# sayands/sgaligner

Hardware: AMD Instinct MI355X
Metric: subscan-pairs/sec (fwd+bwd) + node-match Hits@1 vs reference (higher is better)
Workload: dtype f32 (fp32 operands and fp32 accumulation throughout; the anchors x negatives loss sweeps multiply them as three exact bf16 planes, six bf16 MFMAs per product...

## Files before the change

sgaligner_amd/csrc/sweep3.hip:

```cpp
#include <type_traits>

#include "loss_math.h"

namespace {

typedef __bf16 bf16x8 __attribute__((ext_vector_type(8)));
typedef __bf16 bf16x2 __attribute__((ext_vector_type(2)));
typedef float f32x2 __attribute__((ext_vector_type(2)));
typedef unsigned int u32x4 __attribute__((ext_vector_type(4)));
typedef unsigned int u32x2 __attribute__((ext_vector_type(2)));
typedef short s16x4 __attribute__((ext_vector_type(4)));

constexpr int S3_DP = 104;
constexpr int S3_PLANE = 3 * 2 * 1024;
constexpr int S3_TAIL = 3 * S3_PLANE;
constexpr int S3_BLOCK = S3_TAIL + 2048;
constexpr int S3_NCH = S3_BLOCK / 1024;
constexpr int S3_ROWSLOTS = 3 * 12 + 4;

__device__ __forceinline__ void split3_pair(float v0, float v1, unsigned& h, unsigned& m, unsigned& l) {
    const bf16x2 H = __builtin_convertvector(f32x2{v0, v1}, bf16x2);
    const unsigned hu = __builtin_bit_cast(unsigned, H);
#ifdef S3_SPLIT_DOT2
    unsigned c0 = 0x0000BF80u, c1 = 0xBF800000u;
// ... 82 lines not shown
    if (b < L.nbA) { old0 = 0; len = A; }
    else if (b < 2 * L.nbA) { b -= L.nbA; old0 = A; len = A; }
    else if (b < 2 * L.nbA + L.nb1) { b -= 2 * L.nbA; old0 = 2 * A; len = J1; }
    else { b -= 2 * L.nbA + L.nb1; old0 = 2 * A + J1; len = J2; }
    const int nvalid = min(32, len - 32 * b);
    const float* src = Z + (size_t)(old0 + 32 * b) * S3_DP;
    if (threadIdx.x < S3_DP) zbar[threadIdx.x] = stat[threadIdx.x];
    __syncthreads();
    for (int e = threadIdx.x; e < 32 * S3_DP; e += 256) {
        const int r = e / S3_DP, c = e - r * S3_DP;
        tile[e] = (r < nvalid && c < S3_DREAL) ? src[e] - zbar[c] : 0.f;
        if (Zc && old0 < 2 * A && r < nvalid) Zc[(size_t)(old0 + 32 * b) * S3_DP + e] = c == S3_DREAL + 1 ? 1.f : tile[e];
    }
    __syncthreads();
    if (threadIdx.x < 32) {
        const int r = threadIdx.x;
        if (r < nvalid) {
            double a = 0.0;
            for (int c = 0; c < S3_DREAL; ++c) a += (double)zbar[c] * (double)tile[r * S3_DP + c];
            tile[r * S3_DP + S3_DREAL] = (float)(a + (double)stat[S3_DP]);
            tile[r * S3_DP + S3_DREAL + 1] = 1.f;
        }
    }
    __syncthreads();
    unsigned* out = reinterpret_cast<unsigned*>(Zb + (size_t)blockIdx.x * S3_BLOCK);
    for (int e = threadIdx.x; e < 3 * 2 * 64 * 4; e += 256) {
        const int p = e & 3, st = (e >> 2) & 63, jh = (e >> 8) & 1, q = e >> 9;
        const int g = st >> 4, i = (st & 15) ^ (12 * (g & 1));
        const int row = 8 * (i >> 2) + 4 * jh + (i & 3), col = 32 * q + 8 * g + 2 * p;
        unsigned h, m, l;
        split3_pair(tile[row * S3_DP + col], tile[row * S3_DP + col + 1], h, m, l);
        out[e] = h; out[S3_PLANE / 4 + e] = m; out[2 * S3_PLANE / 4 + e] = l;
    }
    for (int e = threadIdx.x; e < 2 * 64 * 4; e += 256) {
        const int p = e & 3, st = (e >> 2) & 63, jh = (e >> 8) & 1;
        const int g = st >> 4, i = (st & 15) ^ (12 * (g & 1));
        const int row = 8 * (i >> 2) + 4 * jh + (i & 3), col = 96 + 2 * p;
        unsigned h, m, l;
        split3_pair(tile[row * S3_DP + col], tile[row * S3_DP + col + 1], h, m, l);
        out[S3_TAIL / 4 + e] = g < 2 ? h : (g == 2 ? m : l);
    }
}


__global__ __launch_bounds__(256) void centre_tables_kernel(const float* __restrict__ Z, int R, const float* __restrict__ stat, float* __restrict__ Zc) {
    const int lane = threadIdx.x & 63, wpb = blockDim.x >> 6;
    for (int r = blockIdx.x * wpb + (threadIdx.x >> 6); r < R; r += gridDim.x * wpb) {
        const float* z = Z + (size_t)r * S3_DP;
        float* o = Zc + (size_t)r * S3_DP;
        double acc = 0.0;
        float v[2];
#pragma unroll
        for (int t = 0; t < 2; ++t) {
            const int d = lane + 64 * t;
            const float zb = d < S3_DREAL ? stat[d] : 0.f;
            v[t] = d < S3_DREAL ? z[d] - zb : 0.f;
            acc += (double)zb * (double)v[t];
        }
        acc = wave_sum_d(acc);
        o[lane] = v[0];
        const int d1 = lane + 64;
        if (d1 < S3_DP) o[d1] = d1 < S3_DREAL ? v[1] : (d1 == S3_DREAL ? (float)(acc + (double)stat[S3_DP]) : (d1 == S3_DREAL + 1 ? 1.f : 0.f));
    }
}

#ifdef S3_DBG_TIMING
__device__ unsigned long long g_s3_dbg[16];
#define S3_T(i) { const unsigned long long t_ = __builtin_readcyclecounter(); tacc[i] += t_ - tprev; tprev = t_; }
#else
#define S3_T(i)
#endif
struct TSeg { int blk0, jt_lo, jt_hi, old0, lo, hi, fam; };
struct TGroup { int own0, nown, own_old0, own_blk0, blk0, nsplit, nseg; TSeg seg[2]; };
struct TArgs {
    int M; const unsigned char* Zb[4]; int perm[4]; int ngroups; TGroup grp[4];
    float k0, k1, it0, it1, ka;
    const float* beta;
    double* sums;
    const double* gs;
    float* dZ[4];
    double* gamma;
};

template <int M, bool GRAD, int WV, int MG = M, bool GAM = true, bool LITE = false, bool FOLD = false>
__global__ __launch_bounds__(WV * 64, WV == 8 ? 2 : 1) void sweep3_kernel(TArgs a) {
    static_assert(!LITE || !GRAD, "LITE: the forward sums only");
    static_assert(!FOLD || (GRAD && WV == 4), "FOLD: the one-wave-per-SIMD gradient sweep only");
    constexpr int NCT = 7;
    constexpr int WAVES = WV, THREADS = WAVES * 64;
    constexpr int OWN = WV * 16;
    constexpr int NCH = LITE ? S3_NCH - S3_PLANE / 1024 : S3_NCH;
    constexpr int KMAX = (NCH + WAVES - 1) / WAVES;
    constexpr int BUF = M * S3_BLOCK;
    constexpr bool PIPE = WV == 4;
#ifndef S3_OWN_IN_S
#define S3_OWN_IN_S 1
#endif
    constexpr bool OWN_IN_S = GRAD && PIPE && S3_OWN_IN_S;
#ifndef S3_SPREAD
#define S3_SPREAD 1
#endif
    constexpr bool SPREAD = OWN_IN_S && S3_SPREAD && !FOLD;
    extern __shared__ __attribute__((aligned(16))) unsigned char lds3[];

    const int tid = threadIdx.x, lane = tid & 63, wave = tid >> 6, g4 = lane >> 4, l15 = lane & 15;
    int g = 0;
#pragma unroll
    for (int i = 1; i < 4; ++i) if (i < a.ngroups && (int)blockIdx.x >= a.grp[i].blk0) g = i;
    const TGroup& grp = a.grp[g];
    const int wg_in_grp = (int)blockIdx.x - grp.blk0;
    const int nsplit = grp.nsplit, n_ob = (grp.nown + OWN - 1) / OWN, n_units = n_ob * nsplit;
    const int unit = (wg_in_grp & 7) * ((n_units + 7) >> 3) + (wg_in_grp >> 3);
    if ((wg_in_grp >> 3) >= ((n_units + 7) >> 3) || unit >= n_units) return;
    const int split = unit / n_ob;
    const int own0 = grp.own0 + (unit - split * n_ob) * OWN;
    const int own_end = grp.own0 + grp.nown;
    const int wrow0 = own0 + wave * 16;
#ifdef S3_DBG_TIMING
    unsigned long long tacc[8] = {0, 0, 0, 0, 0, 0, 0, 0}, tprev = __builtin_readcyclecounter();
#endif

    u32x4 opl[M][3][3], otl[M][2];
    float beta[M];
    const bool iv = wrow0 + l15 < own_end;
    {
        const int my_i = wrow0 + l15;
        const int rel = (iv ? my_i : own0) - grp.own_old0;
        const int o = rel & 31, oi = 4 * (o >> 3) + (o & 3), ojh = (o >> 2) & 1;
        const size_t off = (size_t)(grp.own_blk0 + (rel >> 5)) * S3_BLOCK;
#pragma unroll
        for (int m = 0; m < M; ++m) {
            const unsigned char* base = a.Zb[m] + off;
#pragma unroll
            for (int p = 0; p < 3; ++p)
#pragma unroll
                for (int q = 0; q < 3; ++q) {
                    const int so = ((q * 2 + ojh) * 64 + s3_slot(g4, oi)) * 16;
                    opl[m][p][q] = iv ? *reinterpret_cast<const u32x4*>(base + p * S3_PLANE + so) : u32x4{0, 0, 0, 0};
                }
            u32x4 th = iv ? *reinterpret_cast<const u32x4*>(base + S3_TAIL + (ojh * 64 + s3_slot(0, oi)) * 16) : u32x4{0, 0, 0, 0};
            u32x4 tm = iv ? *reinterpret_cast<const u32x4*>(base + S3_TAIL + (ojh * 64 + s3_slot(2, oi)) * 16) : u32x4{0, 0, 0, 0};
            u32x4 tl = iv ? *reinterpret_cast<const u32x4*>(base + S3_TAIL + (ojh * 64 + s3_slot(3, oi)) * 16) : u32x4{0, 0, 0, 0};
            const float ksc = a.k1;
            auto rescale = [&](u32x4& ph, u32x4& pm, u32x4& pl) {
#pragma unroll
                for (int d = 0; d < 4; ++d) {
                    const float x0 = (__builtin_bit_cast(float, ph[d] << 16) + __builtin_bit_cast(float, pm[d] << 16)) + __builtin_bit_cast(float, pl[d] << 16);
                    const float x1 = (__builtin_bit_cast(float, ph[d] & 0xffff0000u) + __builtin_bit_cast(float, pm[d] & 0xffff0000u)) + __builtin_bit_cast(float, pl[d] & 0xffff0000u);
                    unsigned nh, nm, nl;
                    split3_pair(x0 * ksc, x1 * ksc, nh, nm, nl);
                    ph[d] = nh; pm[d] = nm; pl[d] = nl;
                }
            };
#pragma unroll
            for (int q = 0; q < 3; ++q) rescale(opl[m][0][q], opl[m][1][q], opl[m][2][q]);
            rescale(th, tm, tl);
            otl[m][0] = g4 == 1 ? tm : th;
            otl[m][1] = g4 == 0 ? tl : (g4 == 2 ? tm : u32x4{0, 0, 0, 0});
#pragma unroll
            for (int t = 0; t < 2; ++t)
                otl[m][t][2] = (otl[m][t][2] >> 16) | (otl[m][t][2] << 16);
        }
    }
#pragma unroll
    for (int m = 0; m < M; ++m) beta[m] = a.beta[a.perm[m]];

    constexpr int NSM = GRAD ? (FOLD ? 1 : MG) : 1;
    f32x4 gacc[GRAD ? MG : 1][NCT], gsm[NSM][NCT];
#pragma unroll
    for (int m = 0; m < (GRAD ? MG : 1); ++m)
#pragma unroll
        for (int ct = 0; ct < NCT; ++ct) gacc[m][ct] = f32x4{0.f, 0.f, 0.f, 0.f};
#pragma unroll
    for (int m = 0; m < NSM; ++m)
#pragma unroll
        for (int ct = 0; ct < NCT; ++ct) gsm[m][ct] = f32x4{0.f, 0.f, 0.f, 0.f};
    float gam[M];
#pragma unroll
    for (int m = 0; m < M; ++m) gam[m] = 0.f;

    const int wave_u = __builtin_amdgcn_readfirstlane(wave);
    unsigned l16 = threadIdx.x;
    asm volatile("" : "+v"(l16));
    l16 = (l16 & 63u) * 16u;
    unsigned long long tb[M];
    auto set_tile = [&](int blk) {
#pragma unroll
        for (int m = 0; m < M; ++m) tb[m] = sreg64(reinterpret_cast<unsigned long long>(a.Zb[m]) + (unsigned long long)blk * S3_BLOCK);
    };
    auto issue_slots = [&](unsigned char* buf, int f_lo, int f_hi) {
#ifdef S3_DBG_NODMA
        return;
#endif
#pragma unroll
        for (int f = f_lo; f < f_hi; ++f) {
            if (f >= M * KMAX) break;
            const int m = f / KMAX, k = f % KMAX;
            const int rot = (wave_u + m) & (WAVES - 1);
            int c = rot + k * WAVES;
            if ((k + 1) * WAVES > NCH) c = c >= NCH ? c - WAVES : c;
            if (LITE) c = c >= 2 * (S3_PLANE / 1024) ? c + S3_PLANE / 1024 : c;
            __builtin_amdgcn_global_load_lds((const __attribute__((address_space(1))) void*)(reinterpret_cast<const unsigned char*>(tb[m] + (unsigned)(c * 1024)) + l16),
                                             (__attribute__((address_space(3))) void*)(buf + m * S3_BLOCK + c * 1024), 16, 0, 0);
        }
    };
    auto issue = [&](int blk, unsigned char* buf) { set_tile(blk); issue_slots(buf, 0, M * KMAX); };

    const int aoff = s3_slot(g4, l15) * 16;
    const int tr_io = 4 * g4 + (l15 >> 2), tr_cs = l15 & 3;
    const int tr_main = s3_slot(tr_cs >> 1, tr_io) * 16 + (tr_cs & 1) * 8;
    const int tr_tail = S3_TAIL + tr_io * 16 + (tr_cs & 1) * 8;
    const int tr_tail_l = S3_TAIL + (48 + (tr_io ^ 12)) * 16 + (tr_cs & 1) * 8;

#pragma unroll 1
    for (int sg = 0; sg < 2; ++sg) {
        if (sg >= grp.nseg) break;
        const TSeg seg = grp.seg[sg];
        float c0[M + 1], c1[M + 1];
#pragma unroll
        for (int m = 0; m <= M; ++m) {
            const int mo = m < M ? a.perm[m] : M;
            c0[m] = GRAD ? (float)(a.gs[mo * 8 + seg.fam * 2 + 0] * (double)a.it0) : 0.f;
            c1[m] = GRAD ? (float)(a.gs[mo * 8 + seg.fam * 2 + 1] * (double)a.it1) : 0.f;
        }
        const float ka = a.ka;
        double dsum[M + 1][2];
#pragma unroll
        for (int m = 0; m <= M; ++m) { dsum[m][0] = 0.0; dsum[m][1] = 0.0; }
        float pl0[LITE ? M + 1 : 1], pl1[LITE ? M + 1 : 1];
#pragma unroll
        for (int m = 0; m < (LITE ? M + 1 : 1); ++m) { pl0[m] = 0.f; pl1[m] = 0.f; }

        __syncthreads();
        if (seg.jt_lo + split < seg.jt_hi) issue(seg.blk0 + seg.jt_lo + split, lds3);
        int it = 0;
#pragma unroll 1
        for (int jt = seg.jt_lo + split; jt < seg.jt_hi; jt += nsplit, ++it) {
            unsigned char* buf = lds3 + (it & 1) * BUF;
            const int j0 = seg.old0 + 32 * jt;
            S3_T(5)
            __syncthreads();
            S3_T(0)
            const int next_blk = seg.blk0 + (jt + nsplit < seg.jt_hi ? jt + nsplit : jt);
            unsigned char* next_buf = lds3 + ((it + 1) & 1) * BUF;
            set_tile(next_blk);
            S3_T(1)
            if (GRAD) {
                const int vlo = max(seg.lo - j0, 0), vhi = min(seg.hi - j0, 32);
                if (vlo > 0 || vhi < 32) {
                    for (int x = tid; x < M * 32 * S3_ROWSLOTS; x += THREADS) {
                        const int pc = x % S3_ROWSLOTS, w = (x / S3_ROWSLOTS) % 32, m = x / (S3_ROWSLOTS * 32);
                        if (w >= vlo && w < vhi) continue;
                        const int wjh = (w >> 2) & 1, wi = 4 * (w >> 3) + (w & 3);
                        unsigned char* base = buf + m * S3_BLOCK;
                        if (pc < 36) {
                            const int pl = pc / 12, q = (pc % 12) >> 2, gq = pc & 3;
                            *reinterpret_cast<u32x4*>(base + pl * S3_PLANE + ((q * 2 + wjh) * 64 + s3_slot(gq, wi)) * 16) = u32x4{0, 0, 0, 0};
                        } else {
                            const int gq = pc - 36;
                            *reinterpret_cast<u32x4*>(base + S3_TAIL + (wjh * 64 + s3_slot(gq, wi)) * 16) = u32x4{0, 0, 0, 0};
                        }
                    }
                    __syncthreads();
                }
            }

            f32x4 sacc[M][2];
            float own[M][2][4];
            float cj[2][4];
            constexpr int NSET = PIPE ? 2 : 1;
            u32x4 at[NSET], ap[NSET][3][3];
            auto ld_one = [&](int ss, int idx) {
                const int e = ss % NSET;
                const unsigned char* ar = buf + (SPREAD ? ss % M : ss >> 1) * S3_BLOCK + (SPREAD ? ss / M : ss & 1) * 1024 + aoff;
                if (idx < 1) at[e] = *reinterpret_cast<const u32x4*>(ar + S3_TAIL);
                else ap[e][2 - (idx - 1) / 3][(idx - 1) % 3] = *reinterpret_cast<const u32x4*>(ar + (2 - (idx - 1) / 3) * S3_PLANE + ((idx - 1) % 3) * 2048);
            };
            auto ld_set = [&](int ss) {
#pragma unroll
                for (int idx = 0; idx < 10; ++idx) if (!(LITE && idx >= 1 && idx <= 3)) ld_one(ss, idx);
            };
            if (PIPE) {
                ld_set(0);
                __builtin_amdgcn_s_waitcnt(0xc07f);
                __builtin_amdgcn_sched_barrier(0);
            }
            if constexpr (SPREAD) {
                constexpr int NDS = 2 * M - 2, PER = (M * KMAX + NDS - 1) / NDS;
                constexpr int PA[6] = {2, 1, 1, 0, 0, 0}, PB[6] = {0, 1, 0, 2, 1, 0};
                f32x4 accp[2][2];
                float ot0 = 0.f, ot1 = 0.f, sjt = 0.f, ce0 = 0.f, ce1 = 0.f;
                auto own_step = [&](int mm, int hh, int r, int k) {
                    const float sv = sacc[mm][hh][r];
                    if (k == 0) ot0 = fexp2(sv * ka);
                    else if (k == 1) ot1 = fexp2(sv);
                    else own[mm][hh][r] = fmaf(c0[mm], ot0, c1[mm] * ot1);
                };
                auto cj_step = [&](int hh, int r, int k) {
                    if (k == 0) {
                        sjt = 0.f;
#pragma unroll
                        for (int mm = 0; mm < M; ++mm) sjt = fmaf(beta[mm], sacc[mm][hh][r], sjt);
                    } else if (k == 1) ce0 = fexp2(sjt * ka);
                    else if (k == 2) ce1 = fexp2(sjt);
                    else cj[hh][r] = c0[M] * ce0 + c1[M] * ce1;
                };
#pragma unroll
                for (int ss = 0; ss < 2 * M; ++ss) {
                    const int m = ss % M, jh = ss / M, e = ss % NSET, pa = ss & 1;
                    const int pm = ss > 0 ? (ss - 1) % M : 0, pjh = ss > 0 ? (ss - 1) / M : 0;
                    accp[pa][0] = f32x4{0.f, 0.f, 0.f, 0.f}; accp[pa][1] = f32x4{0.f, 0.f, 0.f, 0.f};
#pragma unroll
                    for (int x = 0; x < 20; ++x) {
                        if (x == 0) accp[pa][0] = mfma_b(at[e], otl[m][1], accp[pa][0]);
                        else if (x == 1) accp[pa][1] = mfma_b(at[e], otl[m][0], accp[pa][1]);
                        else accp[pa][x & 1] = mfma_b(ap[e][PA[(x - 2) / 3]][(x - 2) % 3], opl[m][PB[(x - 2) / 3]][(x - 2) % 3], accp[pa][x & 1]);
                        __builtin_amdgcn_sched_barrier(0);
                        if (ss + 1 < 2 * M && x < 10) ld_one(ss + 1, x);
                        if (ss < NDS && (x % 3) == 1 && (x / 3) < PER) issue_slots(next_buf, ss * PER + (x / 3), ss * PER + (x / 3) + 1);
                        if (ss > 0) {
                            if (x == 0) { sacc[pm][pjh][0] = accp[pa ^ 1][0][0] + accp[pa ^ 1][1][0]; sacc[pm][pjh][1] = accp[pa ^ 1][0][1] + accp[pa ^ 1][1][1]; }
                            if (x == 2) { sacc[pm][pjh][2] = accp[pa ^ 1][0][2] + accp[pa ^ 1][1][2]; sacc[pm][pjh][3] = accp[pa ^ 1][0][3] + accp[pa ^ 1][1][3]; }
                            if (pm < MG) {
                                constexpr int G0[4] = {3, 8, 12, 16}, G1[4] = {5, 9, 14, 17}, G2[4] = {6, 11, 15, 18};
#pragma unroll
                                for (int r = 0; r < 4; ++r) {
                                    if (x == G0[r]) own_step(pm, pjh, r, 0);
                                    if (x == G1[r]) own_step(pm, pjh, r, 1);
                                    if (x == G2[r]) own_step(pm, pjh, r, 2);
                                }
                            }
                        }
                        if (ss >= NDS) {
                            const int q = (x == 19 ? 5 : (x % 3) == 1 && x <= 13 ? x / 3 : -1);
                            if (q >= 0) {
                                const int qq = (ss - NDS) * 6 + q, r = qq / 3, k = qq % 3;
                                if (k == 0) { if (r > 0) cj_step(0, r - 1, 3); cj_step(0, r, 0); }
                                else cj_step(0, r, k);
                            }
                        }
                        __builtin_amdgcn_sched_barrier(0);
                    }
                }
#pragma unroll
                for (int r = 0; r < 4; ++r) sacc[M - 1][1][r] = accp[(2 * M - 1) & 1][0][r] + accp[(2 * M - 1) & 1][1][r];
                cj_step(0, 3, 3);
            } else {
#pragma unroll
            for (int ss = 0; ss < 2 * M; ++ss) {
                const int m = ss >> 1, jh = ss & 1, e = ss % NSET;
                if (!PIPE) ld_set(ss);
                constexpr int NDS = GRAD ? (2 * M - 2) : 2 * M, PER = (M * KMAX + NDS - 1) / NDS;
                f32x4 acc2[2] = {f32x4{0.f, 0.f, 0.f, 0.f}, f32x4{0.f, 0.f, 0.f, 0.f}};
                float ownt[2] = {0.f, 0.f};
                constexpr int PA[6] = {2, 1, 1, 0, 0, 0}, PB[6] = {0, 1, 0, 2, 1, 0};
#pragma unroll
                for (int x = 0; x < 20; ++x) {
                    const bool skip = LITE && x >= 2 && (PA[(x - 2) / 3] == 2 || PB[(x - 2) / 3] == 2 || (PA[(x - 2) / 3] == 1 && PB[(x - 2) / 3] == 1));
                    if (skip) {}
                    else if (x == 0) acc2[0] = mfma_b(at[e], otl[m][1], acc2[0]);
                    else if (x == 1) acc2[1] = mfma_b(at[e], otl[m][0], acc2[1]);
                    else acc2[x & 1] = mfma_b(ap[e][PA[(x - 2) / 3]][(x - 2) % 3], opl[m][PB[(x - 2) / 3]][(x - 2) % 3], acc2[x & 1]);
                    if (PIPE) {
                        __builtin_amdgcn_sched_barrier(0);
                        if (ss + 1 < 2 * M && x < 10 && !(LITE && x >= 1 && x <= 3)) ld_one(ss + 1, x);
                        if (ss < NDS && (x % 3) == 1 && (x / 3) < PER) issue_slots(next_buf, ss * PER + (x / 3), ss * PER + (x / 3) + 1);
                        if (OWN_IN_S && m > 0 && m - 1 < MG && x >= 11 && x < 19) {
                            const int r = (x - 11) >> 1;
                            const float sv = sacc[m - 1][jh][r];
                            if (((x - 11) & 1) == 0) {
                                ownt[0] = fexp2(sv * ka);
                                ownt[1] = fexp2(sv);
                            } else {
                                own[m - 1][jh][r] = fmaf(c0[m - 1], ownt[0], c1[m - 1] * ownt[1]);
                            }
                        }
                        __builtin_amdgcn_sched_barrier(0);
                    } else if (x == 1 && ss < NDS) {
                        issue_slots(next_buf, ss * PER, (ss + 1) * PER);
                    }
                }
#pragma unroll
                for (int r = 0; r < 4; ++r) sacc[m][jh][r] = acc2[0][r] + acc2[1][r];
            }
            }

            S3_T(2)
            if (!GRAD) {
                float p0[M + 1], p1[M + 1];
#pragma unroll
                for (int m = 0; m <= M; ++m) { p0[m] = LITE ? pl0[LITE ? m : 0] : 0.f; p1[m] = LITE ? pl1[LITE ? m : 0] : 0.f; }
                auto sums_tile = [&](auto masked_c) {
                    constexpr bool MASKED = decltype(masked_c)::value;
#pragma unroll
                    for (int jh = 0; jh < 2; ++jh)
#pragma unroll
                        for (int r = 0; r < 4; ++r) {
                            const int row = j0 + 8 * g4 + 4 * jh + r;
                            const float okf = (!MASKED || (iv && row >= seg.lo && row < seg.hi)) ? 1.f : 0.f;
                            float sj = 0.f;
#pragma unroll
                            for (int m = 0; m < M; ++m) {
                                const float sv = sacc[m][jh][r];
                                sj = fmaf(beta[m], sv, sj);
                                p0[m] = MASKED ? fmaf(okf, fexp2(sv * ka), p0[m]) : p0[m] + fexp2(sv * ka);
                                p1[m] = MASKED ? fmaf(okf, fexp2(sv), p1[m]) : p1[m] + fexp2(sv);
                            }
                            p0[M] = MASKED ? fmaf(okf, fexp2(sj * ka), p0[M]) : p0[M] + fexp2(sj * ka);
                            p1[M] = MASKED ? fmaf(okf, fexp2(sj), p1[M]) : p1[M] + fexp2(sj);
                        }
                };
                if (j0 >= seg.lo && j0 + 32 <= seg.hi && own0 + OWN <= own_end) sums_tile(std::false_type{}); else sums_tile(std::true_type{});
                if (!LITE || (it & 3) == 3) {
#pragma unroll
                    for (int m = 0; m <= M; ++m) { dsum[m][0] += (double)p0[m]; dsum[m][1] += (double)p1[m]; }
#pragma unroll
                    for (int m = 0; m < (LITE ? M + 1 : 1); ++m) { pl0[m] = 0.f; pl1[m] = 0.f; }
                } else {
#pragma unroll
                    for (int m = 0; m < (LITE ? M + 1 : 1); ++m) { pl0[m] = p0[m]; pl1[m] = p1[m]; }
                }
            } else {
                constexpr int BD = PIPE ? 4 : 1;
                u32x4 bp[BD][3];
                auto ld_b = [&](int k) {
                    const int m = k / NCT, ct = k % NCT, par = k % BD;
                    const unsigned char* pb = buf + m * S3_BLOCK;
#pragma unroll
                    for (int p = 0; p < 3; ++p) {
                        const unsigned char* ph = ct < 6 ? pb + p * S3_PLANE + tr_main + (ct >> 1) * 2048 + (ct & 1) * 512
                                                         : pb + (p == 2 ? tr_tail_l : tr_tail + (p == 1 ? 512 : 0));
                        const u32x2 x0 = tr_read16(ph), x1 = tr_read16(ph + 1024);
                        bp[par][p] = u32x4{x0[0], x0[1], x1[0], x1[1]};
                    }
                };
                auto own_last = [&]() {
#pragma unroll
                    for (int r = 0; r < 4; ++r) {
                        const float sv = sacc[M - 1][1][r];
                        own[M - 1][1][r] = fmaf(c0[M - 1], fexp2(sv * ka), c1[M - 1] * fexp2(sv));
                    }
                };
#pragma unroll
                for (int m = SPREAD ? M : OWN_IN_S ? M - 1 : 0; m < MG; ++m)
#pragma unroll
                    for (int jh = 0; jh < 2; ++jh)
#pragma unroll
                        for (int r = 0; r < 4; ++r) {
                            const float sv = sacc[m][jh][r];
#ifdef S3_DBG_NOEPI
                            own[m][jh][r] = sv;
#else
                            own[m][jh][r] = fmaf(c0[m], fexp2(sv * ka), c1[m] * fexp2(sv));
#endif
                        }
#pragma unroll
                for (int jh = SPREAD ? 1 : 0; jh < 2; ++jh)
#pragma unroll
                    for (int r = 0; r < 4; ++r) {
                        float sj = 0.f;
#pragma unroll
                        for (int m = 0; m < M; ++m) sj = fmaf(beta[m], sacc[m][jh][r], sj);
// ... 60 lines not shown
                    __builtin_amdgcn_sched_barrier(0);
                    ld_b(0); ld_b(1);
                    __builtin_amdgcn_sched_barrier(0);
#pragma unroll
                    for (int g4i = 0; g4i < 4 * MG; ++g4i) {
                        const int m = g4i >> 2, ct0 = (g4i & 3) * 2, n = (g4i & 3) == 3 ? 1 : 2, k0_ = NCT * m + ct0;
                        if (SPREAD && g4i == 0 && M - 1 < MG && M > 1) own_last();
                        if ((g4i & 3) == 0 && m + 1 < MG) planes(m + 1);
                        if (GAM && !FOLD && g4i == (MG > 1 ? 4 : 0)) gamma_acc();
                        if (FOLD && g4i >= 2) fold_group(g4i - 2);
                        const int kn = k0_ + n;
                        const int nn = kn >= NCT * MG ? 0 : ((kn % NCT) == 6 ? 1 : 2);
#pragma unroll
                        for (int j = 0; j < nn; ++j) ld_b(kn + j);
                        if (n == 2) {
#pragma unroll
                            for (int i = 0; i < 5; ++i) { step_small(m, ct0, k0_ % BD, i); step_small(m, ct0 + 1, (k0_ + 1) % BD, i); }
                            gacc[GRAD ? m : 0][ct0] = mfma_b(ch[m & 1], bp[k0_ % BD][0], gacc[GRAD ? m : 0][ct0]);
                            gacc[GRAD ? m : 0][ct0 + 1] = mfma_b(ch[m & 1], bp[(k0_ + 1) % BD][0], gacc[GRAD ? m : 0][ct0 + 1]);
                        } else {
                            step_small(m, ct0, k0_ % BD, 0);
                            gacc[GRAD ? m : 0][ct0] = mfma_b(ch[m & 1], bp[k0_ % BD][0], gacc[GRAD ? m : 0][ct0]);
#pragma unroll
                            for (int i = 1; i < 5; ++i) step_small(m, ct0, k0_ % BD, i);
                        }
                        if (FOLD) {
                            if (n == 2) { if (nn == 2) sgb_seq<0, 12, 12, true>(); else if (nn == 1) sgb_seq<0, 12, 6, true>(); else sgb_seq<0, 12, 0, true>(); }
                            else { if (nn == 2) sgb_seq<0, 6, 12, false>(); else if (nn == 1) sgb_seq<0, 6, 6, false>(); else sgb_seq<0, 6, 0, false>(); }
                        } else {
#pragma unroll
                        for (int x = 0; x < 6 * n; ++x) {
                            __builtin_amdgcn_sched_group_barrier(0x008, 1, 0);
                            if (x < 6 * nn) __builtin_amdgcn_sched_group_barrier(0x100, 1, 0);
                            if (n == 2 || x < 2) __builtin_amdgcn_sched_group_barrier(0x002, 2, 0);
                        }
                        }
                        if ((g4i & 3) == 3) __builtin_amdgcn_sched_barrier(0);
                    }
                    if (FOLD) { fold_group(4 * MG - 2); fold_group(4 * MG - 1); }
                }
                S3_T(4)
            }
        }
        if (!GRAD) {
#pragma unroll
            for (int m = 0; m <= M; ++m)
#pragma unroll
                for (int tt = 0; tt < 2; ++tt) {
                    if (LITE) dsum[m][tt] += (double)(tt ? pl1[LITE ? m : 0] : pl0[LITE ? m : 0]);
                    const double v = wave_sum_d(dsum[m][tt]);
                    if (lane == 0 && v != 0.0) atomicAdd(a.sums + (M + 1) * 8 * (1 + my_slot()) + m * 8 + seg.fam * 2 + tt, v);
                }
        }
    }
#ifdef S3_DBG_TIMING
    if (lane == 0) for (int i = 0; i < 8; ++i) atomicAdd(&g_s3_dbg[(GRAD ? 8 : 0) + i], tacc[i]);
#endif
    if (GRAD) {
#pragma unroll
        for (int m = 0; m < MG; ++m) {
            float* dz = a.dZ[m];
#pragma unroll
            for (int ct = 0; ct < NCT; ++ct) if (!FOLD) gacc[GRAD ? m : 0][ct] += gsm[(GRAD && !FOLD) ? m : 0][ct];
#pragma unroll
            for (int ct = 0; ct < NCT; ++ct) {
                const int d = ct * 16 + l15;
                if (d < S3_DREAL || d == S3_DREAL + 1) {
#pragma unroll
                    for (int r = 0; r < 4; ++r) {
                        const int i = wrow0 + 4 * g4 + r;
                        if (i < own_end) atomicAdd(dz + (size_t)i * S3_DP + d, gacc[GRAD ? m : 0][ct][r]);
                    }
                }
            }
        }
        if (GAM && g < 2) {
#pragma unroll
            for (int m = 0; m < M; ++m) {
                const float v = wave_sum(gam[m]) / a.k1;
                if (lane == 0 && v != 0.f) atomicAdd(a.gamma + M * (1 + my_slot()) + a.perm[m], (double)v);
            }
        }
    }
}

struct SProd { const float* S; int ld, tn, own_seg, own0, nown, oth_seg, oth0, noth, blk0, nsplit; };
struct SArgs { const unsigned char* Zb; float* dZ; const float* zero; int A, nbA, n; SProd p[4]; };

__global__ __launch_bounds__(256, 2) void stash3_kernel(SArgs a) {
    constexpr int NCT = 7, WAVES = 4, RW = 2, OWN = WAVES * RW * 16;
    constexpr int KMAX = (S3_NCH + WAVES - 1) / WAVES;
    extern __shared__ __attribute__((aligned(16))) unsigned char lds3[];
    const int tid = threadIdx.x, lane = tid & 63, wave = tid >> 6, g4 = lane >> 4, l15 = lane & 15;
    int pi = 0;
#pragma unroll
    for (int i = 1; i < 4; ++i) if (i < a.n && (int)blockIdx.x >= a.p[i].blk0) pi = i;
    const SProd& P = a.p[pi];
    const float* const PS = P.S;
    const float* const zero_word = a.zero;
    const int Pld = P.ld, Ptn = P.tn, Pnown = P.nown, Poth0 = P.oth0, Pnoth = P.noth;
    const int w_in = (int)blockIdx.x - P.blk0;
    const int n_ob = (P.nown + OWN - 1) / OWN;
    if (w_in >= n_ob * P.nsplit) return;
    const int split = w_in / n_ob, ob = w_in - split * n_ob;
    const int orow0 = ob * OWN + wave * (RW * 16) + l15;
    const int t_lo = P.oth0 >> 5, t_hi = (P.oth0 + P.noth + 31) >> 5;
    const int per = (t_hi - t_lo + P.nsplit - 1) / P.nsplit;
    const int jt0 = t_lo + split * per, jt1 = min(t_hi, jt0 + per);
    if (jt0 >= jt1) return;
    const int oblk0 = P.oth_seg ? a.nbA : 0;

    const int wave_u = __builtin_amdgcn_readfirstlane(wave);
    unsigned l16 = threadIdx.x;
    asm volatile("" : "+v"(l16));
    l16 = (l16 & 63u) * 16u;
    auto issue = [&](int blk, unsigned char* buf) {
        const unsigned long long tb = sreg64(reinterpret_cast<unsigned long long>(a.Zb) + (unsigned long long)blk * S3_BLOCK);
#pragma unroll
        for (int k = 0; k < KMAX; ++k) {
            int c = wave_u + k * WAVES;
            if ((k + 1) * WAVES > S3_NCH) c = c >= S3_NCH ? c - WAVES : c;
            __builtin_amdgcn_global_load_lds((const __attribute__((address_space(1))) void*)(reinterpret_cast<const unsigned char*>(tb + (unsigned)(c * 1024)) + l16),
                                             (__attribute__((address_space(3))) void*)(buf + c * 1024), 16, 0, 0);
        }
    };
    auto load_c = [&](int jt, int rs, float (&c)[8]) {
        const int orow = orow0 + 16 * rs;
        const bool ov = orow < Pnown;
        const int r0 = 32 * jt + 8 * g4 - Poth0;
        if (!Ptn && (Pld & 3) == 0 && (Poth0 & 3) == 0 && ov && r0 >= 0 && r0 + 8 <= Pnoth) {
            const f32x4* q = reinterpret_cast<const f32x4*>(PS + (size_t)orow * Pld + r0);
            const f32x4 u = q[0], v = q[1];
            c[0] = u[0]; c[1] = u[1]; c[2] = u[2]; c[3] = u[3]; c[4] = v[0]; c[5] = v[1]; c[6] = v[2]; c[7] = v[3];
        } else {
            const float* base = PS + (Ptn ? (size_t)orow : (size_t)orow * Pld);
            const int stride = Ptn ? Pld : 1;
            const unsigned lim = ov ? (unsigned)Pnoth : 0u;
#pragma unroll
            for (int k = 0; k < 8; ++k) {
                const int t = r0 + k;
                const bool ok = (unsigned)t < lim;
                const float* q = ok ? base + (size_t)t * stride : zero_word;
                c[k] = *q;
            }
        }
    };

    f32x4 gacc[RW][NCT], gsm[RW][NCT];
#pragma unroll
    for (int rs = 0; rs < RW; ++rs)
#pragma unroll
        for (int ct = 0; ct < NCT; ++ct) { gacc[rs][ct] = f32x4{0.f, 0.f, 0.f, 0.f}; gsm[rs][ct] = f32x4{0.f, 0.f, 0.f, 0.f}; }
    const int tr_io = 4 * g4 + (l15 >> 2), tr_cs = l15 & 3;
    const int tr_main = s3_slot(tr_cs >> 1, tr_io) * 16 + (tr_cs & 1) * 8;
    const int tr_tail = S3_TAIL + tr_io * 16 + (tr_cs & 1) * 8;
    const int tr_tail_l = S3_TAIL + (48 + (tr_io ^ 12)) * 16 + (tr_cs & 1) * 8;

    float c0[RW][8], c1[RW][8];
#pragma unroll
    for (int rs = 0; rs < RW; ++rs) {
        load_c(jt0, rs, c0[rs]);
        if (jt0 + 1 < jt1) load_c(jt0 + 1, rs, c1[rs]);
    }
    issue(oblk0 + jt0, lds3);
    int it = 0;
    auto step = [&](int jt, float (&cc)[RW][8]) {
// ... 12 lines not shown
        if (jt + 2 < jt1) {
#pragma unroll
            for (int rs = 0; rs < RW; ++rs) load_c(jt + 2, rs, cc[rs]);
        }
#pragma unroll
        for (int ct = 0; ct < NCT; ++ct) {
            u32x4 bp[3];
#pragma unroll
            for (int p = 0; p < 3; ++p) {
                const unsigned char* ph = ct < 6 ? buf + p * S3_PLANE + tr_main + (ct >> 1) * 2048 + (ct & 1) * 512
                                                 : buf + (p == 2 ? tr_tail_l : tr_tail + (p == 1 ? 512 : 0));
                const u32x2 x0 = tr_read16(ph), x1 = tr_read16(ph + 1024);
                bp[p] = u32x4{x0[0], x0[1], x1[0], x1[1]};
            }
#pragma unroll
            for (int rs = 0; rs < RW; ++rs) gsm[rs][ct] = mfma_b(cl[rs], bp[0], gsm[rs][ct]);
#pragma unroll
            for (int rs = 0; rs < RW; ++rs) gsm[rs][ct] = mfma_b(ch[rs], bp[2], gsm[rs][ct]);
#pragma unroll
            for (int rs = 0; rs < RW; ++rs) gsm[rs][ct] = mfma_b(cm[rs], bp[1], gsm[rs][ct]);
#pragma unroll
            for (int rs = 0; rs < RW; ++rs) gsm[rs][ct] = mfma_b(cm[rs], bp[0], gsm[rs][ct]);
#pragma unroll
            for (int rs = 0; rs < RW; ++rs) gsm[rs][ct] = mfma_b(ch[rs], bp[1], gsm[rs][ct]);
#pragma unroll
            for (int rs = 0; rs < RW; ++rs) gacc[rs][ct] = mfma_b(ch[rs], bp[0], gacc[rs][ct]);
        }
        ++it;
    };
#pragma unroll 1
    for (int jt = jt0; jt < jt1; jt += 2) {
        step(jt, c0);
        if (jt + 1 < jt1) step(jt + 1, c1);
    }
    float* dz = a.dZ + (size_t)(P.own_seg ? a.A : 0) * S3_DP;
#pragma unroll
    for (int rs = 0; rs < RW; ++rs)
#pragma unroll
        for (int ct = 0; ct < NCT; ++ct) {
            const int d = ct * 16 + l15;
            if (d < S3_DREAL || d == S3_DREAL + 1) {
#pragma unroll
                for (int r = 0; r < 4; ++r) {
                    const int o = ob * OWN + wave * (RW * 16) + 16 * rs + 4 * g4 + r;
                    if (o < P.nown) atomicAdd(dz + (size_t)(P.own0 + o) * S3_DP + d, gacc[rs][ct][r] + gsm[rs][ct][r]);
                }
            }
        }
}

int fill_t(TArgs& a, const void* const* Zb, int M, const float* beta, int A, int J1, int J2, float tau0, float tau1, bool grad,
           int a_lo, int a_hi, int own_rows, const char* who) {
    if (M < 2 || M > 4) { sga_set_error("%s: M=%d (the three-plane bf16 sweeps are built for 2, 3 or 4 modality tables)", who, M); return SGA_ERR_ARG; }
    if (a_lo < 0 || a_hi > A || a_lo > a_hi) { sga_set_error("%s: anchor shard [%d,%d) outside [0,%d]", who, a_lo, a_hi, A); return SGA_ERR_ARG; }
    a.M = M;
    const TLayout L = make_tlayout(A, J1, J2);
    for (int m = 0; m < M; ++m) {
        if (!Zb[m]) { sga_set_error("%s: null table", who); return SGA_ERR_ARG; }
        a.Zb[m] = static_cast<const unsigned char*>(Zb[m]);
        a.perm[m] = m;
    }
    a.beta = beta; a.k0 = LOG2E / tau0; a.k1 = LOG2E / tau1; a.it0 = 1.f / tau0; a.it1 = 1.f / tau1; a.ka = a.k0 / a.k1;
    const int ns = a_hi - a_lo;
    const int bx1 = 0, bx2 = L.nbA, bn1 = 2 * L.nbA, bn2 = 2 * L.nbA + L.nb1;
    const int ox1 = 0, ox2 = A, on1 = 2 * A, on2 = 2 * A + J1;
    const TSeg N1a{bn1, 0, L.nb1, on1, on1, on1 + J1, 0}, N2a{bn2, 0, L.nb2, on2, on2, on2 + J2, 1};
    const TSeg N2b{bn2, 0, L.nb2, on2, on2, on2 + J2, 2}, N1b{bn1, 0, L.nb1, on1, on1, on1 + J1, 3};
    int g = 0;
    auto add = [&](int own0, int nown, int own_old0, int own_blk0, TSeg s0, TSeg s1) {
        if (nown <= 0) return;
        TGroup& G = a.grp[g++];
        G.own0 = own0; G.nown = nown; G.own_old0 = own_old0; G.own_blk0 = own_blk0; G.nseg = 2; G.seg[0] = s0; G.seg[1] = s1; G.nsplit = 1; G.blk0 = 0;
    };
    add(ox1 + a_lo, ns, ox1, bx1, N1a, N2a);
    add(ox2 + a_lo, ns, ox2, bx2, N2b, N1b);
    if (grad) {
        const int jl = a_lo / 32, jh = (a_hi + 31) / 32;
        const TSeg X1f0{bx1, jl, jh, ox1, ox1 + a_lo, ox1 + a_hi, 0}, X2f3{bx2, jl, jh, ox2, ox2 + a_lo, ox2 + a_hi, 3};
        const TSeg X1f1{bx1, jl, jh, ox1, ox1 + a_lo, ox1 + a_hi, 1}, X2f2{bx2, jl, jh, ox2, ox2 + a_lo, ox2 + a_hi, 2};
        add(on1, J1, on1, bn1, X1f0, X2f3);
        add(on2, J2, on2, bn2, X1f1, X2f2);
    }
    a.ngroups = g;
    int nwg = 0;
    for (int i = 0; i < g; ++i) {
        TGroup& G = a.grp[i];
        int steps = 0;
        for (int sg = 0; sg < G.nseg; ++sg) steps += G.seg[sg].jt_hi - G.seg[sg].jt_lo;
        const long n_ob_g = (G.nown + own_rows - 1) / own_rows;
        const long want = (long)steps * n_ob_g / (12L * sga_num_cus());
        const int unit_steps = want < 160 ? 160 : want > 640 ? 640 : (int)want;
        int nsp = (steps + unit_steps - 1) / unit_steps;
        if (nsp > steps) nsp = steps;
        if (nsp < 1) nsp = 1;
        G.nsplit = nsp;
        G.blk0 = nwg;
        nwg += (((G.nown + own_rows - 1) / own_rows) * nsp + 7) / 8 * 8;
    }
    return -nwg;
}

#ifndef S3_WV_SUMS
#define S3_WV_SUMS 8
#endif
#ifndef S3_WV_GRAD3
#define S3_WV_GRAD3 4
#endif
#ifndef S3_WV_GRAD2
#define S3_WV_GRAD2 4
#endif
template <int M, bool GRAD> constexpr int s3_wv() { return M == 4 ? 4 : GRAD ? (M == 3 ? S3_WV_GRAD3 : S3_WV_GRAD2) : S3_WV_SUMS; }

template <int M, bool GRAD, int MG = M, bool GAM = true, bool LITE = false, bool FOLD = false>
void launch_t(const TArgs& a, int nwg, hipStream_t s) {
    constexpr int WV = s3_wv<M, GRAD>();
    const size_t lds = (size_t)2 * M * S3_BLOCK;
    auto k = sweep3_kernel<M, GRAD, WV, MG, GAM, LITE, FOLD>;
    hipFuncSetAttribute(reinterpret_cast<const void*>(k), hipFuncAttributeMaxDynamicSharedMemorySize, (int)lds);
    hipLaunchKernelGGL(k, dim3(nwg), dim3(WV * 64), lds, s, a);
}

}

#ifdef S3_DBG_TIMING
extern "C" int sga_dbg_sweep3(unsigned long long* host16) {
    if (hipMemcpyFromSymbol(host16, HIP_SYMBOL(g_s3_dbg), sizeof(g_s3_dbg)) != hipSuccess) return 1;
    static unsigned long long z[16];
    return hipMemcpyToSymbol(HIP_SYMBOL(g_s3_dbg), z, sizeof(z)) != hipSuccess;
}
#endif

extern "C" size_t sga_loss_split3_bytes(int A, int J1, int J2) {
    const TLayout L = make_tlayout(A, J1, J2);
    return (size_t)(2 * L.nbA + L.nb1 + L.nb2 + 1) * S3_BLOCK + S3_STAT_BYTES + (size_t)S3_CS_BLOCKS * S3_DP * sizeof(double);
}

extern "C" int sga_loss_split3_tables(const float* Z, int A, int J1, int J2, void* Zb, float* Zc, void* stream) {
    SGA_CHECK_ARG(A >= 0 && J1 >= 0 && J2 >= 0, "sga_loss_split3_tables: bad sizes");
    const TLayout L = make_tlayout(A, J1, J2);
    const int nb = 2 * L.nbA + L.nb1 + L.nb2;
    if (nb == 0) return SGA_OK;
    SGA_CHECK_ARG(Z && Zb, "sga_loss_split3_tables: null pointer");
    hipStream_t s = static_cast<hipStream_t>(stream);
    unsigned char* tail = static_cast<unsigned char*>(Zb) + (size_t)nb * S3_BLOCK;
    if (hipMemsetAsync(tail, 0, S3_BLOCK + S3_STAT_BYTES, s) != hipSuccess) { sga_set_error("sga_loss_split3_tables: memset failed"); return SGA_ERR_HIP; }
    float* stat = reinterpret_cast<float*>(tail + S3_BLOCK);
    double* part = reinterpret_cast<double*>(tail + S3_BLOCK + S3_STAT_BYTES);
    const int R = 2 * A + J1 + J2;
    const int ncs = R < 64 * S3_CS_BLOCKS ? (R + 63) / 64 : S3_CS_BLOCKS;
    hipLaunchKernelGGL(split3_colsum_kernel, dim3(ncs), dim3(128), 0, s, Z, R, part);
    hipLaunchKernelGGL(split3_stats_kernel, dim3(1), dim3(128), 0, s, part, ncs, R, stat);
    hipLaunchKernelGGL(split3_tables_kernel, dim3(nb), dim3(256), 0, s, Z, A, J1, J2, static_cast<unsigned char*>(Zb), stat, Zc);
    SGA_CHECK_LAUNCH("sga_loss_split3_tables");
    return SGA_OK;
}

extern "C" size_t sga_loss_centre_bytes(void) { return S3_STAT_BYTES + (size_t)S3_CS_BLOCKS * S3_DP * sizeof(double); }

extern "C" int sga_loss_centre_tables(const float* Z, int A, int J1, int J2, float* Zc, void* stat_ws, void* stream) {
    SGA_CHECK_ARG(A >= 0 && J1 >= 0 && J2 >= 0, "sga_loss_centre_tables: bad sizes");
    const int R = 2 * A + J1 + J2;
    SGA_CHECK_ARG(stat_ws, "sga_loss_centre_tables: null statistics workspace");
    hipStream_t s = static_cast<hipStream_t>(stream);
    if (hipMemsetAsync(stat_ws, 0, S3_STAT_BYTES, s) != hipSuccess) { sga_set_error("sga_loss_centre_tables: memset failed"); return SGA_ERR_HIP; }
    if (R == 0) return SGA_OK;
    SGA_CHECK_ARG(Z && Zc, "sga_loss_centre_tables: null pointer");
// ... 161 lines not shown
```

Baseline: 974.8.

## Stage tiles with buffer-resource loads to LDS and specialise gamma-free groups

Global-to-LDS tile copies now go through per-segment buffer resource descriptors with scalar offsets instead of 64-bit global pointers. Per-chunk rotation offsets are precomputed, which drops per-issue address arithmetic. Explicit waitcnt barriers are added at each substep, and the kernel body is templated so groups 2 and 3 run a variant compiled without gamma accumulation. A host check rejects segments whose descriptor range would exceed 4 GiB, and the explicit waits could stall the pipeline more than before.

```diff
diff --git a/sgaligner_amd/csrc/sweep3.hip b/sgaligner_amd/csrc/sweep3.hip
--- a/sgaligner_amd/csrc/sweep3.hip
+++ b/sgaligner_amd/csrc/sweep3.hip
@@ -188,8 +188,8 @@
     double* gamma;
 };
 
-template <int M, bool GRAD, int WV, int MG = M, bool GAM = true, bool LITE = false, bool FOLD = false>
-__global__ __launch_bounds__(WV * 64, WV == 8 ? 2 : 1) void sweep3_kernel(TArgs a) {
+template <int M, bool GRAD, int WV, int MG, bool GAM, bool LITE, bool FOLD>
+__device__ __forceinline__ void sweep3_body(const TArgs& a, const int g) {
     static_assert(!LITE || !GRAD, "LITE: the forward sums only");
     static_assert(!FOLD || (GRAD && WV == 4), "FOLD: the one-wave-per-SIMD gradient sweep only");
     constexpr int NCT = 7;
@@ -210,9 +210,6 @@
     extern __shared__ __attribute__((aligned(16))) unsigned char lds3[];
 
     const int tid = threadIdx.x, lane = tid & 63, wave = tid >> 6, g4 = lane >> 4, l15 = lane & 15;
-    int g = 0;
-#pragma unroll
-    for (int i = 1; i < 4; ++i) if (i < a.ngroups && (int)blockIdx.x >= a.grp[i].blk0) g = i;
     const TGroup& grp = a.grp[g];
     const int wg_in_grp = (int)blockIdx.x - grp.blk0;
     const int nsplit = grp.nsplit, n_ob = (grp.nown + OWN - 1) / OWN, n_units = n_ob * nsplit;
@@ -286,31 +283,56 @@
     for (int m = 0; m < M; ++m) gam[m] = 0.f;
 
     const int wave_u = __builtin_amdgcn_readfirstlane(wave);
-    unsigned l16 = threadIdx.x;
-    asm volatile("" : "+v"(l16));
-    l16 = (l16 & 63u) * 16u;
-    unsigned long long tb[M];
-    auto set_tile = [&](int blk) {
-#pragma unroll
-        for (int m = 0; m < M; ++m) tb[m] = sreg64(reinterpret_cast<unsigned long long>(a.Zb[m]) + (unsigned long long)blk * S3_BLOCK);
+    const unsigned l16 = (threadIdx.x & 63u) * 16u;
+    __amdgpu_buffer_rsrc_t rs[M];
+    typedef __attribute__((address_space(3))) unsigned char* lds_ptr;
+    constexpr bool LAST_ODD = KMAX * WAVES > NCH || (LITE && KMAX * WAVES > 2 * (S3_PLANE / 1024));
+    unsigned crot[M], clast[M], trot[M], brot[M];
+    unsigned tile_off = 0, buf_off = 0;
+#pragma unroll
+    for (int m = 0; m < M; ++m) {
+        const int rot = (wave_u + m) & (WAVES - 1);
+        int c = rot + (KMAX - 1) * WAVES;
+        c = c >= NCH ? c - WAVES : c;
+        if (LITE) c = c >= 2 * (S3_PLANE / 1024) ? c + S3_PLANE / 1024 : c;
+        crot[m] = (unsigned)rot * 1024u; clast[m] = (unsigned)c * 1024u;
+        trot[m] = 0; brot[m] = 0;
+    }
+    auto set_seg = [&](const TSeg& sgm) {
+#pragma unroll
+        for (int m = 0; m < M; ++m)
+            rs[m] = __builtin_amdgcn_make_buffer_rsrc(const_cast<unsigned char*>(a.Zb[m]) + (size_t)sgm.blk0 * S3_BLOCK, (short)0,
+                                                      (int)((unsigned)sgm.jt_hi * (unsigned)S3_BLOCK), 0x00020000);
     };
-    auto issue_slots = [&](unsigned char* buf, int f_lo, int f_hi) {
+    auto set_tile = [&](int jt, unsigned char* buf) {
+        tile_off = (unsigned)jt * (unsigned)S3_BLOCK;
+        buf_off = (unsigned)(buf - lds3);
+#pragma unroll
+        for (int m = 0; m < M; ++m) {
+            trot[m] = tile_off + crot[m]; brot[m] = buf_off + (unsigned)(m * S3_BLOCK) + crot[m];
+            asm("" : "+s"(trot[m]), "+s"(brot[m]));
+        }
+    };
+    auto issue_slots = [&](int f_lo, int f_hi) {
 #ifdef S3_DBG_NODMA
         return;
+#endif
+#ifdef S3_DBG_DMA_WAVES
+        unsigned dma_mask = S3_DBG_DMA_WAVES;
+        asm volatile("" : "+s"(dma_mask));
+        if (!((dma_mask >> wave_u) & 1u)) return;
 #endif
 #pragma unroll
         for (int f = f_lo; f < f_hi; ++f) {
             if (f >= M * KMAX) break;
             const int m = f / KMAX, k = f % KMAX;
-            const int rot = (wave_u + m) & (WAVES - 1);
-            int c = rot + k * WAVES;
-            if ((k + 1) * WAVES > NCH) c = c >= NCH ? c - WAVES : c;
-            if (LITE) c = c >= 2 * (S3_PLANE / 1024) ? c + S3_PLANE / 1024 : c;
-            __builtin_amdgcn_global_load_lds((const __attribute__((address_space(1))) void*)(reinterpret_cast<const unsigned char*>(tb[m] + (unsigned)(c * 1024)) + l16),
-                                             (__attribute__((address_space(3))) void*)(buf + m * S3_BLOCK + c * 1024), 16, 0, 0);
+            unsigned so, lo;
+            if (LAST_ODD && k == KMAX - 1) { so = tile_off + clast[m]; lo = buf_off + (unsigned)(m * S3_BLOCK) + clast[m]; }
+            else { so = trot[m] + (unsigned)(k * WAVES * 1024); lo = brot[m] + (unsigned)(k * WAVES * 1024); }
+            __builtin_amdgcn_raw_ptr_buffer_load_lds(rs[m], (lds_ptr)lds3 + lo, 16, l16, so, 0, 0);
         }
     };
-    auto issue = [&](int blk, unsigned char* buf) { set_tile(blk); issue_slots(buf, 0, M * KMAX); };
+    auto issue = [&](int jt, unsigned char* buf) { set_tile(jt, buf); issue_slots(0, M * KMAX); };
 
     const int aoff = s3_slot(g4, l15) * 16;
     const int tr_io = 4 * g4 + (l15 >> 2), tr_cs = l15 & 3;
@@ -322,6 +344,7 @@
     for (int sg = 0; sg < 2; ++sg) {
         if (sg >= grp.nseg) break;
         const TSeg seg = grp.seg[sg];
+        set_seg(seg);
         float c0[M + 1], c1[M + 1];
 #pragma unroll
         for (int m = 0; m <= M; ++m) {
@@ -338,7 +361,7 @@
         for (int m = 0; m < (LITE ? M + 1 : 1); ++m) { pl0[m] = 0.f; pl1[m] = 0.f; }
 
         __syncthreads();
-        if (seg.jt_lo + split < seg.jt_hi) issue(seg.blk0 + seg.jt_lo + split, lds3);
+        if (seg.jt_lo + split < seg.jt_hi) issue(seg.jt_lo + split, lds3);
         int it = 0;
 #pragma unroll 1
         for (int jt = seg.jt_lo + split; jt < seg.jt_hi; jt += nsplit, ++it) {
@@ -347,9 +370,9 @@
             S3_T(5)
             __syncthreads();
             S3_T(0)
-            const int next_blk = seg.blk0 + (jt + nsplit < seg.jt_hi ? jt + nsplit : jt);
+            const int next_jt = jt + nsplit < seg.jt_hi ? jt + nsplit : jt;
             unsigned char* next_buf = lds3 + ((it + 1) & 1) * BUF;
-            set_tile(next_blk);
+            set_tile(next_jt, next_buf);
             S3_T(1)
             if (GRAD) {
                 const int vlo = max(seg.lo - j0, 0), vhi = min(seg.hi - j0, 32);
@@ -374,6 +397,9 @@
             f32x4 sacc[M][2];
             float own[M][2][4];
             float cj[2][4];
+            auto substep_wait = [&](int ss) {
+                if (ss > 0) { __builtin_amdgcn_s_waitcnt(0xc07f); __builtin_amdgcn_sched_barrier(0); }
+            };
             constexpr int NSET = PIPE ? 2 : 1;
             u32x4 at[NSET], ap[NSET][3][3];
             auto ld_one = [&](int ss, int idx) {
@@ -416,6 +442,7 @@
                     const int m = ss % M, jh = ss / M, e = ss % NSET, pa = ss & 1;
                     const int pm = ss > 0 ? (ss - 1) % M : 0, pjh = ss > 0 ? (ss - 1) / M : 0;
                     accp[pa][0] = f32x4{0.f, 0.f, 0.f, 0.f}; accp[pa][1] = f32x4{0.f, 0.f, 0.f, 0.f};
+                    substep_wait(ss);
 #pragma unroll
                     for (int x = 0; x < 20; ++x) {
                         if (x == 0) accp[pa][0] = mfma_b(at[e], otl[m][1], accp[pa][0]);
@@ -423,7 +450,7 @@
                         else accp[pa][x & 1] = mfma_b(ap[e][PA[(x - 2) / 3]][(x - 2) % 3], opl[m][PB[(x - 2) / 3]][(x - 2) % 3], accp[pa][x & 1]);
                         __builtin_amdgcn_sched_barrier(0);
                         if (ss + 1 < 2 * M && x < 10) ld_one(ss + 1, x);
-                        if (ss < NDS && (x % 3) == 1 && (x / 3) < PER) issue_slots(next_buf, ss * PER + (x / 3), ss * PER + (x / 3) + 1);
+                        if (ss < NDS && (x % 3) == 1 && (x / 3) < PER) issue_slots(ss * PER + (x / 3), ss * PER + (x / 3) + 1);
                         if (ss > 0) {
                             if (x == 0) { sacc[pm][pjh][0] = accp[pa ^ 1][0][0] + accp[pa ^ 1][1][0]; sacc[pm][pjh][1] = accp[pa ^ 1][0][1] + accp[pa ^ 1][1][1]; }
                             if (x == 2) { sacc[pm][pjh][2] = accp[pa ^ 1][0][2] + accp[pa ^ 1][1][2]; sacc[pm][pjh][3] = accp[pa ^ 1][0][3] + accp[pa ^ 1][1][3]; }
@@ -456,6 +483,7 @@
             for (int ss = 0; ss < 2 * M; ++ss) {
                 const int m = ss >> 1, jh = ss & 1, e = ss % NSET;
                 if (!PIPE) ld_set(ss);
+                if (PIPE) substep_wait(ss);
                 constexpr int NDS = GRAD ? (2 * M - 2) : 2 * M, PER = (M * KMAX + NDS - 1) / NDS;
                 f32x4 acc2[2] = {f32x4{0.f, 0.f, 0.f, 0.f}, f32x4{0.f, 0.f, 0.f, 0.f}};
                 float ownt[2] = {0.f, 0.f};
@@ -470,7 +498,7 @@
                     if (PIPE) {
                         __builtin_amdgcn_sched_barrier(0);
                         if (ss + 1 < 2 * M && x < 10 && !(LITE && x >= 1 && x <= 3)) ld_one(ss + 1, x);
-                        if (ss < NDS && (x % 3) == 1 && (x / 3) < PER) issue_slots(next_buf, ss * PER + (x / 3), ss * PER + (x / 3) + 1);
+                        if (ss < NDS && (x % 3) == 1 && (x / 3) < PER) issue_slots(ss * PER + (x / 3), ss * PER + (x / 3) + 1);
                         if (OWN_IN_S && m > 0 && m - 1 < MG && x >= 11 && x < 19) {
                             const int r = (x - 11) >> 1;
                             const float sv = sacc[m - 1][jh][r];
@@ -483,7 +511,7 @@
                         }
                         __builtin_amdgcn_sched_barrier(0);
                     } else if (x == 1 && ss < NDS) {
-                        issue_slots(next_buf, ss * PER, (ss + 1) * PER);
+                        issue_slots(ss * PER, (ss + 1) * PER);
                     }
                 }
 #pragma unroll
@@ -710,6 +738,19 @@
             }
         }
     }
+}
+
+template <int M, bool GRAD, int WV, int MG = M, bool GAM = true, bool LITE = false, bool FOLD = false>
+__global__ __launch_bounds__(WV * 64, WV == 8 ? 2 : 1) void sweep3_kernel(TArgs a) {
+    int g = 0;
+#pragma unroll
+    for (int i = 1; i < 4; ++i) if (i < a.ngroups && (int)blockIdx.x >= a.grp[i].blk0) g = i;
+#ifndef S3_GAM_ALL
+    if constexpr (GRAD && GAM) {
+        if (g >= 2) { sweep3_body<M, GRAD, WV, MG, false, LITE, FOLD>(a, g); return; }
+    }
+#endif
+    sweep3_body<M, GRAD, WV, MG, GAM, LITE, FOLD>(a, g);
 }
 
 struct SProd { const float* S; int ld, tn, own_seg, own0, nown, oth_seg, oth0, noth, blk0, nsplit; };
@@ -888,6 +929,12 @@
         add(on2, J2, on2, bn2, X1f1, X2f2);
     }
     a.ngroups = g;
+    for (int i = 0; i < g; ++i)
+        for (int sg = 0; sg < a.grp[i].nseg; ++sg)
+            if ((long long)a.grp[i].seg[sg].jt_hi * S3_BLOCK >= (1LL << 32)) {
+                sga_set_error("%s: a segment of %d 32-row blocks exceeds the 4 GiB a copy descriptor spans", who, a.grp[i].seg[sg].jt_hi);
+                return SGA_ERR_ARG;
+            }
     int nwg = 0;
     for (int i = 0; i < g; ++i) {
         TGroup& G = a.grp[i];
```

Measured after the change: 986.2 (median of 6 runs). 1.01x the previous value.
